# smdogroup/eigd

Measured on AMD Instinct MI355X. Metric: adjoint_mode_derivatives_per_sec, higher is better.
Workload: dtype f64

## Files before the change

eigd_amd/csrc/factor.hip:

```cpp
#include <algorithm>
#include <cstdlib>
#include <cstring>
#include <mutex>

#include "common.h"
#include "symbolic.h"

struct eigd_symbolic {
  eigd::Symbolic s;
  std::mutex upper_lock;
};

static bool ensure_upper_map(eigd_symbolic* h) {
  std::lock_guard<std::mutex> g(h->upper_lock);
  return eigd::build_upper_map(h->s);
}

namespace eigd {

constexpr int TW = 64;
constexpr int TLD = TW + 1;
constexpr int kFragWavesFwd = 2, kFragWaves = 3, kFragWavesBwd32 = 2, kThinWavesLeaf = 3, kThinWavesKids = 1;
constexpr int KBMAX = 32;

struct FrontArrays {
  const int* c0;
  const int* ns;
  const int* bs;
  const int* parent;
  const int64_t* foff;
  const int64_t* voff;
  const int64_t* ioff;
  const int64_t* bptr;
  const int* rel;
  const int64_t* toff;
  int nslot;
  int64_t vrows;
  const int* v_src;
  const int* cmask;
  const int* bout;
  double* sgn;
  const double* zero;
  const int* neg1;
  int W;
  int tri;
  double pivtol;
};

constexpr int kPlaneCols = 4 + 8 + 16 + 32;
constexpr int kMaxS = 4;

__device__ __forceinline__ int find_slot(const int* __restrict__ pref, int na, int idx) {
  int lo = 0, hi = na;
  while (hi - lo > 1) {
    const int mid = (lo + hi) >> 1;
    if (pref[mid] <= idx)
      lo = mid;
    else
      hi = mid;
  }
  return lo;
}

__global__ void scatter_a_kernel(int64_t nlower, const int64_t* __restrict__ src, const int64_t* __restrict__ dst,
                                 const double* __restrict__ data, double* __restrict__ F) {
  for (int64_t e = static_cast<int64_t>(blockIdx.x) * blockDim.x + threadIdx.x; e < nlower;
       e += static_cast<int64_t>(gridDim.x) * blockDim.x)
    F[dst[e]] = data[src[e]];
}

__global__ __launch_bounds__(kThreads) void absmax_kernel(int64_t n, const double* __restrict__ x, double* __restrict__ partial) {
  __shared__ double red[kThreads];
  double m = 0.0;
  for (int64_t i = static_cast<int64_t>(blockIdx.x) * kThreads + threadIdx.x; i < n; i += static_cast<int64_t>(gridDim.x) * kThreads)
    m = fmax(m, fabs(x[i]));
  red[threadIdx.x] = m;
  __syncthreads();
  for (int s = kThreads / 2; s > 0; s >>= 1) {
    if (threadIdx.x < s) red[threadIdx.x] = fmax(red[threadIdx.x], red[threadIdx.x + s]);
    __syncthreads();
  }
  if (threadIdx.x == 0) partial[blockIdx.x] = red[0];
}

__global__ __launch_bounds__(kThreads) void extend_add_kernel(FrontArrays fa, const int* __restrict__ children,
                                                             double* __restrict__ F) {
  const int c = children[blockIdx.x];
  const int p = fa.parent[c];
  const int ns = fa.ns[c], bs = fa.bs[c];
  const int64_t dc = ns + bs, dp = fa.ns[p] + fa.bs[p];
  const int* __restrict__ rel = fa.rel + fa.bptr[c];
  const double* __restrict__ Fc = F + fa.foff[c] + static_cast<int64_t>(ns) * dc + ns;
  double* Fp = F + fa.foff[p];
  const int total = bs * bs;
  for (int idx = blockIdx.y * kThreads + threadIdx.x; idx < total; idx += gridDim.y * kThreads) {
    const int j = idx / bs, i = idx - j * bs;
    if (i >= j) Fp[static_cast<int64_t>(rel[j]) * dp + rel[i]] += Fc[static_cast<int64_t>(j) * dc + i];
  }
}

__global__ __launch_bounds__(kThreads) void potrf_inv_kernel(FrontArrays fa, const int* __restrict__ fronts, int step,
                                                            double* __restrict__ F, double* __restrict__ Inv,
                                                            int* __restrict__ flag) {
  __shared__ double S[TW * TLD];
  __shared__ double Iv[TW * TLD];
// ... 569 lines not shown
    }
    __syncthreads();
    double out[4][4];
#pragma unroll
    for (int p = 0; p < 4; ++p)
#pragma unroll
      for (int q = 0; q < 4; ++q) out[p][q] = 0.0;
    for (int kk = 0; kk < wi; ++kk) {
      double a[4], b[4];
#pragma unroll
      for (int q = 0; q < 4; ++q) a[q] = As[kk * TLD + r0 + q];
#pragma unroll
      for (int q = 0; q < 4; ++q) b[q] = Bs[kk * TLD + c0 + q];
#pragma unroll
      for (int p = 0; p < 4; ++p)
#pragma unroll
        for (int q = 0; q < 4; ++q) out[p][q] += a[p] * b[q];
    }
#pragma unroll
    for (int q = 0; q < 4; ++q)
#pragma unroll
      for (int p = 0; p < 4; ++p)
        if (r0 + p < wi && c0 + q < wj) Tf[static_cast<int64_t>(j0 + c0 + q) * ns + i0 + r0 + p] = -out[p][q];
    __threadfence();
    __syncthreads();
  }
}

__global__ __launch_bounds__(kThreads) void m21_kernel(FrontArrays fa, const int* __restrict__ m_pref, int nfronts,
                                                      double* F, const double* __restrict__ Tb) {
  __shared__ double As[TW * TLD];
  __shared__ double Bs[TW * TLD];
  const int f = find_slot(m_pref, nfronts, blockIdx.x);
  const int bt = blockIdx.x - m_pref[f];
  const int ns = fa.ns[f];
  const int64_t d = ns + fa.bs[f];
  const int rb0 = ns + bt * TW;
  const int rows = min(TW, static_cast<int>(d) - rb0);
  const int nct = (ns + TW - 1) / TW;
  double* Ff = F + fa.foff[f];
  const double* Tf = Tb + fa.toff[f];
  const int tid = threadIdx.x;
  const int r0 = (tid % 16) * 4, c0 = (tid / 16) * 4;
  for (int jt = 0; jt < nct; ++jt) {
    const int j0 = jt * TW, wj = min(TW, ns - j0);
    double acc[4][4];
#pragma unroll
    for (int a = 0; a < 4; ++a)
#pragma unroll
      for (int b = 0; b < 4; ++b) acc[a][b] = 0.0;
    for (int kt = jt; kt < nct; ++kt) {
      const int k0 = kt * TW, wk = min(TW, ns - k0);
      for (int idx = tid; idx < TW * TW; idx += kThreads) {
        const int kk = idx / TW, r = idx - kk * TW;
        As[kk * TLD + r] = (kk < wk && r < rows) ? Ff[static_cast<int64_t>(k0 + kk) * d + rb0 + r] : 0.0;
      }
      for (int idx = tid; idx < TW * TW; idx += kThreads) {
        const int c = idx / TW, kk = idx - c * TW;
        Bs[kk * TLD + c] = (kk < wk && c < wj) ? Tf[static_cast<int64_t>(j0 + c) * ns + k0 + kk] : 0.0;
      }
      __syncthreads();
      for (int kk = 0; kk < wk; ++kk) {
        double a[4], b[4];
#pragma unroll
        for (int q = 0; q < 4; ++q) a[q] = As[kk * TLD + r0 + q];
#pragma unroll
        for (int q = 0; q < 4; ++q) b[q] = Bs[kk * TLD + c0 + q];
#pragma unroll
        for (int p = 0; p < 4; ++p)
#pragma unroll
          for (int q = 0; q < 4; ++q) acc[p][q] += a[p] * b[q];
      }
      __syncthreads();
    }
#pragma unroll
    for (int q = 0; q < 4; ++q)
#pragma unroll
      for (int p = 0; p < 4; ++p)
        if (r0 + p < rows && c0 + q < wj) Ff[static_cast<int64_t>(j0 + c0 + q) * d + rb0 + r0 + p] = acc[p][q];
  }
}


template <int KPT>
struct Tile {
  static constexpr bool kMfma = (KPT >= 4);
  static constexpr int KB = 4 * KPT;
  static constexpr int NT = kMfma ? KB / 16 : 1;
  static constexpr int BLD = (KB == 32) ? 48 : KB;
  static constexpr int NOUT = kMfma ? 4 * NT : KPT;

  __device__ static __forceinline__ void coords(int t, int& row, int& col) {
    if (kMfma) {
      const int lane = threadIdx.x & 63, wave = threadIdx.x >> 6;
      row = 16 * wave + (lane >> 4) + 4 * (t & 3);
      col = 16 * (t >> 2) + (lane & 15);
    } else {
      row = threadIdx.x >> 2;
      col = (threadIdx.x & 3) * KPT + t;
    }
  }

  __device__ static __forceinline__ void mac(const double* __restrict__ As, const double* __restrict__ Bs, int kdim,
                                             double (&acc)[NOUT]) {
    if constexpr (kMfma) {
      const int lane = threadIdx.x & 63, wave = threadIdx.x >> 6;
      const int li = lane & 15, lk = lane >> 4;
      const int o = 16 * wave + li;
      double4_t c[NT];
#pragma unroll
      for (int n = 0; n < NT; ++n) c[n] = double4_t{acc[4 * n], acc[4 * n + 1], acc[4 * n + 2], acc[4 * n + 3]};
      const int kd = (kdim + 7) & ~7;
      for (int k0 = 0; k0 < kd; k0 += 8) {
#pragma unroll
        for (int kk = 0; kk < 8; kk += 4) {
          const int k = k0 + kk + lk;
          const double a = As[k * TLD + o];
#pragma unroll
          for (int n = 0; n < NT; ++n)
            c[n] = __builtin_amdgcn_mfma_f64_16x16x4f64(a, Bs[k * BLD + 16 * n + li], c[n], 0, 0, 0);
        }
      }
#pragma unroll
      for (int n = 0; n < NT; ++n)
#pragma unroll
        for (int r = 0; r < 4; ++r) acc[4 * n + r] = c[n][r];
    } else {
      const int o = threadIdx.x >> 2, cg = threadIdx.x & 3;
      const int kd = (kdim + 7) & ~7;
      for (int k0 = 0; k0 < kd; k0 += 8) {
#pragma unroll
        for (int kk = 0; kk < 8; ++kk) {
          const int k = k0 + kk;
          const double a = As[k * TLD + o];
          const double* b = Bs + k * BLD + cg * KPT;
#pragma unroll
          for (int q = 0; q < KPT; ++q) acc[q] += a * b[q];
        }
      }
    }
  }
};

struct WgRec {
  int f, tile, s0, s1;
  int slab, cnt, G, flags;
  int ns, bs, c0, slot;
  int64_t voff, foff, toff, bptr;
  int64_t pvoff;
  int64_t scratch;
  int64_t ftoff;
  int64_t ldt;
  int64_t moff;
};

struct FragFront {
  int f, nst, nbt, nko;
  int nkb, pad;
  int64_t fm, bm;
};

__device__ __host__ inline int64_t frag_fwd_steps(int nst, int nko, int rt) {
  const int64_t ks = 16 * (nst - 1) + nko;
  return (rt <= nst - 1) ? 8LL * rt * (rt + 1) : 8LL * (nst - 1) * nst + ks * (rt - (nst - 1));
}
__device__ __host__ inline int64_t frag_bwd_chain(int nst, int nbt, int nko, int nkb, int ct) {
// ... 1 lines not shown
}
__device__ __host__ inline int64_t frag_bwd_steps(int nst, int nbt, int nko, int nkb, int ct) {
  int64_t sum = 0;
  for (int c = 0; c < ct; ++c) sum += frag_bwd_chain(nst, nbt, nko, nkb, c);
  return sum;
}
__device__ __host__ inline int64_t frag_bwd_in_chain(int nown, int nko, int t) {
  return (t < nown) ? 16LL * t : 16LL * (nown - 1) + nko + 16LL * (t - nown);
}

struct LevelArgs {
  const WgRec* wg;
  double* P;
  int* tickets;
  int kb;
  int kd;
  int nwg;
  int per_xcd;
  double* V1;
};

__device__ __forceinline__ int xcd_record(const LevelArgs& la) {
  if (la.per_xcd == 0) return blockIdx.x;
  return (blockIdx.x & 7) * la.per_xcd + (blockIdx.x >> 3);
}

constexpr int TILE_IT = TW * TW / kThreads;

__global__ void overflow_sum_kernel(int nrows, const int* __restrict__ ov_dst, const int* __restrict__ ov_ptr,
                                    const int* __restrict__ ov_src, int kb, int ld, double* __restrict__ extra,
                                    const double* __restrict__ scratch) {
  const int idx = blockIdx.x * blockDim.x + threadIdx.x;
  if (idx >= nrows * kb) return;
  const int x = idx / kb, c = idx - x * kb;
  double sum = 0.0;
  for (int e = ov_ptr[x]; e < ov_ptr[x + 1]; ++e) sum += scratch[static_cast<int64_t>(ov_src[e]) * ld + c];
  extra[static_cast<int64_t>(ov_dst[x]) * ld + c] = sum;
}

template <int KPT>
__device__ __forceinline__ bool fold_groups(const WgRec& w, const LevelArgs& la, double (&acc)[Tile<KPT>::NOUT],
                                            int* sflag) {
  using T = Tile<KPT>;
  typedef unsigned long long u64;
  double* Pp = la.P + static_cast<int64_t>(w.slab) * (TW * KBMAX);
  u64* mine = reinterpret_cast<u64*>(Pp + static_cast<int64_t>(w.flags >> 8) * (TW * KBMAX));
#pragma unroll
  for (int t = 0; t < T::NOUT; ++t)
    __hip_atomic_store(mine + t * kThreads + threadIdx.x, static_cast<u64>(__double_as_longlong(acc[t])),
                       __ATOMIC_RELAXED, __HIP_MEMORY_SCOPE_AGENT);
  asm volatile("s_waitcnt vmcnt(0)" ::: "memory");
  __syncthreads();
  if (threadIdx.x == 0)
    *sflag = (__hip_atomic_fetch_add(la.tickets + w.cnt, 1, __ATOMIC_RELAXED, __HIP_MEMORY_SCOPE_AGENT) == w.G - 1) ? 1 : 0;
  __syncthreads();
  if (*sflag == 0) return false;
  if (threadIdx.x == 0) {
    __hip_atomic_store(la.tickets + w.cnt, 0, __ATOMIC_RELAXED, __HIP_MEMORY_SCOPE_AGENT);
    __builtin_amdgcn_fence(__ATOMIC_ACQUIRE, "agent");
    asm volatile("s_waitcnt vmcnt(0)" ::: "memory");
  }
  __syncthreads();
#pragma unroll
  for (int t = 0; t < T::NOUT; ++t) acc[t] = 0.0;
  for (int gg = 0; gg < w.G; gg += 2) {
    const double* p0 = Pp + static_cast<int64_t>(gg) * (TW * KBMAX) + threadIdx.x;
    const bool two = gg + 1 < w.G;
    double a[T::NOUT], b[T::NOUT];
#pragma unroll
    for (int t = 0; t < T::NOUT; ++t) {
      a[t] = p0[t * kThreads];
      b[t] = two ? p0[TW * KBMAX + t * kThreads] : 0.0;
    }
#pragma unroll
    for (int t = 0; t < T::NOUT; ++t) {
      acc[t] += a[t];
      if (two) acc[t] += b[t];
    }
  }
  return true;
}

template <int KPT, bool SINGLE, int NSL, bool FRAG = false, bool PRE = false>
__global__ __launch_bounds__(kThreads) __attribute__((amdgpu_waves_per_eu(((SINGLE && KPT >= 4) || (FRAG && KPT >= 4)) ? ((FRAG && KPT >= 8) ? kFragWavesFwd : 3) : 1)))
void fwd_level_kernel(FrontArrays fa, LevelArgs la, const double* __restrict__ F,
                                                            const double* __restrict__ Tb, const double* X, int ldx,
                                                            double alpha, double* V, double* __restrict__ Y) {
  using T = Tile<KPT>;
  constexpr int IT = KPT;
  extern __shared__ double lds_tiles[];
  double* const As = lds_tiles;
  const int kdl = SINGLE ? la.kd : TW;
  double* const Bs = lds_tiles + (((SINGLE && KPT == 4) || FRAG) ? 0 : (kdl + 1) * TLD);
  const int rec = SINGLE ? static_cast<int>(blockIdx.x) : xcd_record(la);
  if (!SINGLE && rec >= la.nwg) return;
  const WgRec w = la.wg[rec];
  const int kb = la.kb;
  const int ns = w.ns;
  const int d = ns + w.bs;
  const int nst = (ns + TW - 1) / TW;
  const bool kids = (w.flags & 2) != 0;
  const int64_t vbase = w.voff;
  const double* Tf = Tb + w.toff;
  const double* Ff = F + w.foff;
  const int ar = threadIdx.x & (TW - 1), ajb = threadIdx.x >> 6;

  int xi[IT];
  double bv[IT], av[TILE_IT];
  const int nslot = kids ? fa.nslot : 0;
  const int64_t vslot = fa.vrows * T::KB;
  double* Vout = V + static_cast<int64_t>(w.slot) * vslot;

  static_assert(!PRE || FRAG, "pre-assembled right-hand sides: the fragment path only");
  auto fetch_idx = [&](int ct) {
    if constexpr (PRE) return;
    const int wd = min(TW, ns - ct * TW);
#pragma unroll
    for (int e = 0; e < IT; ++e) {
      const int r = (threadIdx.x + e * kThreads) / T::KB;
      const int64_t vrow = vbase + ct * TW + r;
      const bool ok = r < wd;
      xi[e] = *(ok ? fa.v_src + vrow : fa.neg1);
    }
  };
  auto fetch_b = [&](int ct) {
    if constexpr (PRE) {
      const int wd = min(TW, ns - ct * TW);
      const double* V1 = la.V1 + (vbase + ct * TW) * T::KB;
#pragma unroll
      for (int e = 0; e < IT; ++e) {
        const int idx = threadIdx.x + e * kThreads;
        bv[e] = *(((idx & (T::KB - 1)) < kb && idx / T::KB < wd) ? V1 + idx : fa.zero);
      }
      return;
    }
#pragma unroll
    for (int e = 0; e < IT; ++e) {
      const int idx = threadIdx.x + e * kThreads;
      const int c = idx & (T::KB - 1);
      const bool ok = c < kb && xi[e] >= 0;
      const double xv = alpha * *(ok ? X + static_cast<int64_t>(xi[e]) * ldx + c : fa.zero);
      const double* cp = V + (vbase + ct * TW + idx / T::KB) * T::KB + c;
      double v = 0.0;
#pragma unroll
      for (int s = 0; s < NSL; ++s) v += *((ok && s < nslot) ? cp + s * vslot : fa.zero);
      bv[e] = xv + v;
    }
  };
  auto fetch_a = [&](int rt, int ct, double (&av)[TILE_IT]) {
    const bool own = rt < nst;
    const int row0 = own ? rt * TW : ns + (rt - nst) * TW;
    const int rows = min(TW, (own ? ns : d) - row0);
    const int64_t ld = own ? w.ldt : d;
    const int wd = min(TW, ns - ct * TW);
    const double* Ap = (own ? Tf : Ff) + static_cast<int64_t>(ct) * TW * ld + row0 + ar;
#pragma unroll
    for (int it = 0; it < TILE_IT; ++it) {
      const int j = ajb + it * (kThreads / TW);
      av[it] = *((j < wd && ar < rows) ? Ap + static_cast<int64_t>(j) * ld : fa.zero);
    }
  };
  auto commit_a = [&](const double (&av)[TILE_IT]) {
#pragma unroll
    for (int it = 0; it < TILE_IT; ++it)
      As[min(ajb + it * (kThreads / TW), kdl) * TLD + ar] = av[it];
  };
  auto commit_b = [&]() {
// ... 74 lines not shown
      const double* Ab = (own ? Tf : Ff) + row0;
      const ptrdiff_t zoff = fa.zero - Ab;
#pragma unroll
      for (int kk = 0; kk < 16; ++kk) {
        const int k = 4 * kk + lk;
        a[kk] = (k < ns && orow < rows) ? Ab[static_cast<unsigned>(k * ld + orow)] : Ab[zoff];
      }
    };
    auto stepd = [&](int rt, double (&cur)[16], int nxt) {
      if (KPT < 8 && rt >= nst) fetch_carry(rt, cg, di);
      double4_t c[T::NT];
#pragma unroll
      for (int n = 0; n < T::NT; ++n) c[n] = double4_t{0.0, 0.0, 0.0, 0.0};
#pragma unroll
      for (int kk = 0; kk < 16; ++kk) {
        const int k = 4 * kk + lk;
#pragma unroll
        for (int n = 0; n < T::NT; ++n)
          c[n] = __builtin_amdgcn_mfma_f64_16x16x4f64(cur[kk], Bs[k * T::BLD + 16 * n + li], c[n], 0, 0, 0);
      }
      if (nxt < w.s1) fetch_frag(nxt, cur);
#pragma unroll
      for (int n = 0; n < T::NT; ++n)
#pragma unroll
        for (int r = 0; r < 4; ++r) acc[4 * n + r] = c[n][r];
      if (KPT >= 8 && rt >= nst) fetch_carry(rt, cg, di);
      store_tile(rt, acc, cg, di);
    };
    double a0[16];
    fetch_idx(0);
    fetch_frag(w.s0, a0);
    constexpr int HB = (IT > 4) ? IT / 2 : IT;
#pragma unroll
    for (int h = 0; h < IT; h += HB) {
      double vh[HB];
#pragma unroll
      for (int e = h; e < h + HB; ++e) {
        const int idx = threadIdx.x + e * kThreads;
        const int c = idx & (T::KB - 1);
        const bool ok = c < kb && xi[e] >= 0;
        const double xv = alpha * *(ok ? X + static_cast<int64_t>(xi[e]) * ldx + c : fa.zero);
        const double* cp = V + (vbase + idx / T::KB) * T::KB + c;
        double v = 0.0;
#pragma unroll
        for (int s = 0; s < NSL; ++s) v += *((ok && s < nslot) ? cp + s * vslot : fa.zero);
        vh[e - h] = xv + v;
      }
#pragma unroll
      for (int e = h; e < h + HB; ++e) {
        const int idx = threadIdx.x + e * kThreads;
        Bs[min(idx / T::KB, kdl) * T::BLD + (idx & (T::KB - 1))] = vh[e - h];
      }
      asm volatile("" ::: "memory");
    }
    __syncthreads();
    for (int rt = w.s0; rt < w.s1; ++rt) stepd(rt, a0, rt + 1);
  } else if constexpr (SINGLE) {
    auto step = [&](int rt, double (&cur)[TILE_IT], int nxt) {
      commit_a(cur);
      __syncthreads();
      if (nxt < w.s1) fetch_a(nxt, 0, cur);
      if (rt >= nst) fetch_carry(rt, cg, di);
#pragma unroll
      for (int t = 0; t < T::NOUT; ++t) acc[t] = 0.0;
      T::mac(As, Bs, ns, acc);
      store_tile(rt, acc, cg, di);
      __syncthreads();
    };
    fetch_idx(0);
    fetch_b(0);
    fetch_a(w.s0, 0, av);
    commit_b();
    for (int rt = w.s0; rt < w.s1; ++rt) step(rt, av, rt + 1);
  } else if constexpr (FRAG) {
    static_assert(!FRAG || T::kMfma, "fragments feed MFMAs");
    const int wave = threadIdx.x >> 6, lane = threadIdx.x & 63;
    const int li = lane & 15, lk = lane >> 4;
    const int rt = w.tile;
    const bool own = rt < nst;
    const int row0 = own ? rt * TW : ns + (rt - nst) * TW;
    const int rows = min(TW, (own ? ns : d) - row0);
    const bool wok = 16 * wave < rows;
    const double* Am = F + w.moff + wave * 64 + lane;
    auto fetch_frag = [&](int ct, double (&a)[16]) {
      const int nk = (min(TW, ns - ct * TW) + 3) >> 2;
      const double* Ac = Am + static_cast<int64_t>(ct) * (TW * TW);
#pragma unroll
      for (int kk = 0; kk < 16; ++kk) a[kk] = (wok && kk < nk) ? Ac[kk * 256] : 0.0;
    };
    double4_t c[T::NT];
#pragma unroll
    for (int n = 0; n < T::NT; ++n) c[n] = double4_t{0.0, 0.0, 0.0, 0.0};
    auto stepf = [&](int ct, double (&cur)[16], double (&nxt)[16]) {
      commit_b();
      __syncthreads();
      if (ct + 1 < w.s1) {
        fetch_b(ct + 1);
        fetch_frag(ct + 1, nxt);
        if (ct + 2 < w.s1) fetch_idx(ct + 2);
      }
      const int nk = (min(TW, ns - ct * TW) + 3) >> 2;
#pragma unroll
      for (int kk = 0; kk < 16; ++kk) {
        if (kk < nk) {
          const int k = 4 * kk + lk;
#pragma unroll
          for (int n = 0; n < T::NT; ++n)
            c[n] = __builtin_amdgcn_mfma_f64_16x16x4f64(cur[kk], Bs[k * T::BLD + 16 * n + li], c[n], 0, 0, 0);
        }
      }
      __syncthreads();
    };
    double a0[16], a1[16];
    fetch_frag(w.s0, a0);
    fetch_idx(w.s0);
    fetch_b(w.s0);
    if (w.s0 + 1 < w.s1) fetch_idx(w.s0 + 1);
    for (int ct = w.s0; ct < w.s1; ct += 2) {
      stepf(ct, a0, a1);
      if (ct + 1 < w.s1) stepf(ct + 1, a1, a0);
    }
#pragma unroll
    for (int n = 0; n < T::NT; ++n)
#pragma unroll
      for (int r = 0; r < 4; ++r) acc[4 * n + r] = c[n][r];
    if (rt >= nst) fetch_carry(rt, cg, di);
    if (w.G > 1 && !fold_groups<KPT>(w, la, acc, reinterpret_cast<int*>(Bs))) return;
    store_tile(rt, acc, cg, di);
  } else {
  const int rt = w.tile;
  fetch_idx(w.s0);
  fetch_b(w.s0);
  fetch_a(rt, w.s0, av);
  if (w.s0 + 1 < w.s1) fetch_idx(w.s0 + 1);
  for (int ct = w.s0; ct < w.s1; ++ct) {
    commit_a(av);
    commit_b();
    __syncthreads();
    if (ct + 1 < w.s1) {
      fetch_b(ct + 1);
      fetch_a(rt, ct + 1, av);
      if (ct + 2 < w.s1) fetch_idx(ct + 2);
    }
    T::mac(As, Bs, min(TW, ns - ct * TW), acc);
    __syncthreads();
  }
  if (rt >= nst) fetch_carry(rt, cg, di);
  if (w.G > 1 && !fold_groups<KPT>(w, la, acc, reinterpret_cast<int*>(As))) return;
  store_tile(rt, acc, cg, di);
  }
}

template <int KPT, int NSL>
__global__ __launch_bounds__(kThreads) void v1_assemble_kernel(FrontArrays fa, const WgRec* __restrict__ recs, const double* X,
                                                              int ldx, double alpha, const double* V, double* V1p, int kb) {
  using T = Tile<KPT>;
  constexpr int IT = KPT;
  const WgRec w = recs[blockIdx.x];
  const int ct = w.tile;
  const int wd = min(TW, w.ns - ct * TW);
  const int64_t vrow0 = w.voff + ct * TW;
  const int nslot = ((w.flags & 2) != 0) ? fa.nslot : 0;
  const int64_t vslot = fa.vrows * T::KB;
  int xi[IT];
#pragma unroll
  for (int e = 0; e < IT; ++e) {
    const int r = (threadIdx.x + e * kThreads) / T::KB;
    xi[e] = *((r < wd) ? fa.v_src + vrow0 + r : fa.neg1);
  }
  double bv[IT];
#pragma unroll
  for (int e = 0; e < IT; ++e) {
    const int idx = threadIdx.x + e * kThreads;
    const int c = idx & (T::KB - 1);
    const bool ok = c < kb && xi[e] >= 0;
    const double xv = alpha * *(ok ? X + static_cast<int64_t>(xi[e]) * ldx + c : fa.zero);
    const double* cp = V + vrow0 * T::KB + idx;
    double v = 0.0;
#pragma unroll
    for (int s = 0; s < NSL; ++s) v += *((ok && s < nslot) ? cp + s * vslot : fa.zero);
    bv[e] = xv + v;
  }
  double* V1 = V1p + vrow0 * T::KB;
#pragma unroll
  for (int e = 0; e < IT; ++e) {
    const int idx = threadIdx.x + e * kThreads;
    if ((idx & (T::KB - 1)) < kb && xi[e] >= 0) V1[idx] = bv[e];
  }
}

constexpr int kLidxMax = 7168;
template <int KPT, bool SINGLE, bool FRAG = false, bool LIDX = false>
__global__ __launch_bounds__(kThreads) __attribute__((amdgpu_waves_per_eu(FRAG ? (KPT >= 8 ? (LIDX ? 3 : kFragWavesBwd32) : kFragWaves) : 1)))
void bwd_level_kernel(FrontArrays fa, LevelArgs la, const double* __restrict__ F,
                                                            const double* __restrict__ Tb, const double* __restrict__ Ft,
                                                            const double* __restrict__ Y, double* Out, int ldo) {
  using T = Tile<KPT>;
  constexpr int IT = KPT;
  extern __shared__ double lds_tiles[];
  double* const As = lds_tiles;
  const int kdl = SINGLE ? la.kd : TW;
  double* const Bs = lds_tiles + (FRAG ? 0 : (kdl + 1) * TLD);
  const int rec = SINGLE ? static_cast<int>(blockIdx.x) : xcd_record(la);
  if (!SINGLE && rec >= la.nwg) return;
  const WgRec w = la.wg[rec];
  const int ct = w.tile;
  const int kb = la.kb;
  const int ns = w.ns, bs = w.bs;
  const int d = ns + bs;
  const int nst = (ns + TW - 1) / TW;
  const int c0t = ct * TW;
  const int wc = min(TW, ns - c0t);
  const int nown = nst - ct;
  const int64_t vbase = w.voff;
  const double* Tp = Tb + w.toff + static_cast<int64_t>(c0t) * w.ldt;
  const double* Mp = F + w.foff + static_cast<int64_t>(c0t) * d;
  const int* __restrict__ bout = fa.bout + w.bptr;
  const int ar = threadIdx.x & (TW - 1), ajb = threadIdx.x >> 6;

  int ri[IT];
  double bv[IT], av[TILE_IT];
  int pend_rows = 0;

  auto fetch_idx = [&](int t) {
    if (t < nown) return;
    const int b0 = (t - nown) * TW;
    const int rows = min(TW, bs - b0);
#pragma unroll
    for (int e = 0; e < IT; ++e) {
      const int r = (threadIdx.x + e * kThreads) / T::KB;
      ri[e] = *((r < rows) ? bout + b0 + r : fa.neg1);
    }
  };
  auto fetch_val = [&](int t) {
    const bool border = t >= nown;
    const int rbase = border ? ns + (t - nown) * TW : (ct + t) * TW;
    const int rows = min(TW, (border ? d : ns) - rbase);
    if (!border) {
      const double* Yp = Y + (vbase + rbase) * kb;
#pragma unroll
      for (int e = 0; e < IT; ++e) {
        const int idx = threadIdx.x + e * kThreads;
        const int r = idx / T::KB, c = idx & (T::KB - 1);
        bv[e] = *((r < rows && c < kb) ? Yp + static_cast<int64_t>(r) * kb + c : fa.zero);
      }
    } else {
#pragma unroll
      for (int e = 0; e < IT; ++e) {
        const int c = (threadIdx.x + e * kThreads) & (T::KB - 1);
        bv[e] = -*((ri[e] >= 0 && c < kb) ? Out + static_cast<int64_t>(ri[e]) * ldo + c : fa.zero);
      }
    }
    const double* Ap = (border ? Mp : Tp) + rbase + ar;
    const int64_t ld = border ? d : w.ldt;
#pragma unroll
    for (int it = 0; it < TILE_IT; ++it) {
      const int j = ajb + it * (kThreads / TW);
      av[it] = *((j < wc && ar < rows) ? Ap + static_cast<int64_t>(j) * ld : fa.zero);
    }
    pend_rows = rows;
  };
  auto commit = [&]() {
#pragma unroll
    for (int it = 0; it < TILE_IT; ++it)
      As[min(ar, kdl) * TLD + ajb + it * (kThreads / TW)] = av[it];
#pragma unroll
    for (int e = 0; e < IT; ++e) {
      const int idx = threadIdx.x + e * kThreads;
      Bs[min(idx / T::KB, kdl) * T::BLD + (idx & (T::KB - 1))] = bv[e];
    }
  };

  double acc[T::NOUT];
  int oi[T::NOUT];
#pragma unroll
  for (int t = 0; t < T::NOUT; ++t) acc[t] = 0.0;
  if constexpr (FRAG) {
    static_assert(!FRAG || (!SINGLE && T::kMfma), "fragments: several column tiles, MFMA widths");
    const int wave = threadIdx.x >> 6, lane = threadIdx.x & 63;
    const int li = lane & 15, lk = lane >> 4;
    const bool wok = 16 * wave < wc;
    const int nko = (ns - TW * (nst - 1) + 3) >> 2;
    const double* Am = Ft + w.moff + wave * 64 + lane;
    int frag_rows = 0;
    static_assert(!LIDX || FRAG, "index list in LDS: the fragment path only");
    int* const Is = reinterpret_cast<int*>(Bs + (TW + 1) * T::BLD);
    auto fetch_vec = [&](int t) {
      const bool border = t >= nown;
      const int rbase = border ? ns + (t - nown) * TW : (ct + t) * TW;
      const int rows = min(TW, (border ? d : ns) - rbase);
      if (!border) {
        const double* Yp = Y + (vbase + rbase) * kb;
#pragma unroll
        for (int e = 0; e < IT; ++e) {
          const int idx = threadIdx.x + e * kThreads;
          const int r = idx / T::KB, c = idx & (T::KB - 1);
          bv[e] = *((r < rows && c < kb) ? Yp + static_cast<int64_t>(r) * kb + c : fa.zero);
        }
      } else if constexpr (LIDX) {
        const int b0 = (t - nown) * TW;
        int rr[IT];
#pragma unroll
        for (int e = 0; e < IT; ++e) {
          const int r = (threadIdx.x + e * kThreads) / T::KB;
          rr[e] = (r < rows) ? Is[b0 + r] : -1;
        }
#pragma unroll
        for (int e = 0; e < IT; ++e) {
          const int c = (threadIdx.x + e * kThreads) & (T::KB - 1);
          bv[e] = -*((rr[e] >= 0 && c < kb) ? Out + static_cast<int64_t>(rr[e]) * ldo + c : fa.zero);
        }
      } else {
#pragma unroll
        for (int e = 0; e < IT; ++e) {
          const int c = (threadIdx.x + e * kThreads) & (T::KB - 1);
          bv[e] = -*((ri[e] >= 0 && c < kb) ? Out + static_cast<int64_t>(ri[e]) * ldo + c : fa.zero);
        }
      }
    };
    auto fetch_frag = [&](int t, double (&a)[16]) {
      const bool border = t >= nown;
      const int rbase = border ? ns + (t - nown) * TW : (ct + t) * TW;
      const int rows = min(TW, (border ? d : ns) - rbase);
      const int nk = (rows + 3) >> 2;
      const double* Ac = Am + 256 * frag_bwd_in_chain(nown, nko, t);
#pragma unroll
      for (int kk = 0; kk < 16; ++kk) a[kk] = (wok && kk < nk) ? Ac[kk * 256] : 0.0;
      frag_rows = rows;
    };
    auto commit_vec = [&]() {
#pragma unroll
      for (int e = 0; e < IT; ++e) {
        const int idx = threadIdx.x + e * kThreads;
        Bs[(idx / T::KB) * T::BLD + (idx & (T::KB - 1))] = bv[e];
      }
    };
    double4_t c[T::NT];
#pragma unroll
    for (int n = 0; n < T::NT; ++n) c[n] = double4_t{0.0, 0.0, 0.0, 0.0};
    auto stepb = [&](int t, double (&cur)[16], double (&nxt)[16]) {
      const int nk = (frag_rows + 3) >> 2;
      commit_vec();
      __syncthreads();
      if (t + 1 < w.s1) {
        fetch_vec(t + 1);
        fetch_frag(t + 1, nxt);
        if (!LIDX && t + 2 < w.s1) fetch_idx(t + 2);
      }
#pragma unroll
      for (int kk = 0; kk < 16; ++kk) {
        if (kk < nk) {
          const int k = 4 * kk + lk;
#pragma unroll
          for (int n = 0; n < T::NT; ++n)
            c[n] = __builtin_amdgcn_mfma_f64_16x16x4f64(cur[kk], Bs[k * T::BLD + 16 * n + li], c[n], 0, 0, 0);
        }
      }
      __syncthreads();
    };
    double a0[16], a1[16];
    fetch_frag(w.s0, a0);
    if constexpr (LIDX) {
      constexpr int NI = 8;
      int ib[NI];
      const bool any = w.s1 > nown;
#pragma unroll
      for (int q = 0; q < NI; ++q) ib[q] = *((any && threadIdx.x + q * kThreads < bs) ? bout + threadIdx.x + q * kThreads : fa.neg1);
      if (w.s0 < nown) fetch_vec(w.s0);
#pragma unroll
      for (int q = 0; q < NI; ++q)
        if (any && threadIdx.x + q * kThreads < bs) Is[threadIdx.x + q * kThreads] = ib[q];
      if (any)
        for (int i = NI * kThreads + threadIdx.x; i < bs; i += kThreads) Is[i] = bout[i];
      if (w.s0 >= nown) {
        __syncthreads();
        fetch_vec(w.s0);
      }
    } else {
      fetch_idx(w.s0);
      fetch_vec(w.s0);
      if (w.s0 + 1 < w.s1) fetch_idx(w.s0 + 1);
    }
    for (int t = w.s0; t < w.s1; t += 2) {
      stepb(t, a0, a1);
      if (t + 1 < w.s1) stepb(t + 1, a1, a0);
    }
#pragma unroll
    for (int n = 0; n < T::NT; ++n)
#pragma unroll
      for (int r = 0; r < 4; ++r) acc[4 * n + r] = c[n][r];
  } else {
  fetch_idx(w.s0);
  fetch_val(w.s0);
  if (w.s0 + 1 < w.s1) fetch_idx(w.s0 + 1);
  for (int t = w.s0; t < w.s1; ++t) {
    const int kdim = pend_rows;
    commit();
    __syncthreads();
    if (t + 1 < w.s1) {
      fetch_val(t + 1);
      if (t + 2 < w.s1) fetch_idx(t + 2);
    }
    T::mac(As, Bs, kdim, acc);
    __syncthreads();
  }
  }
#pragma unroll
  for (int t = 0; t < T::NOUT; ++t) {
    int o, c;
    T::coords(t, o, c);
    oi[t] = *((o < wc && c < kb) ? fa.v_src + vbase + c0t + o : fa.neg1);
  }
  if (w.G > 1 && !fold_groups<KPT>(w, la, acc, reinterpret_cast<int*>(lds_tiles))) return;
  __builtin_amdgcn_s_waitcnt(0x0F70);
#pragma unroll
  for (int t = 0; t < T::NOUT; ++t) {
    int o, c;
    T::coords(t, o, c);
    if (oi[t] >= 0) Out[static_cast<int64_t>(oi[t]) * ldo + c] = acc[t];
  }
}

__device__ __forceinline__ double readlane_f64(double v, int l) {
  const int lo = __builtin_amdgcn_readlane(__double2loint(v), l);
  const int hi = __builtin_amdgcn_readlane(__double2hiint(v), l);
  return __hiloint2double(hi, lo);
}

template <int KB, int NSL, int WPF>
__global__ __launch_bounds__(64 * WPF) void fwd_wave_kernel(FrontArrays fa, const WgRec* __restrict__ recs,
                                                       const double* __restrict__ F, const double* __restrict__ Tb,
                                                       const double* X, int ldx, double alpha, double* V,
                                                       double* __restrict__ Y, int kb) {
  const WgRec w = recs[blockIdx.x];
  const int lane = threadIdx.x & 63, wave = threadIdx.x >> 6;
  const int ns = w.ns, d = ns + w.bs;
  const bool kids = (w.flags & 2) != 0;
  const int nslot = kids ? fa.nslot : 0;
  const int64_t vslot = fa.vrows * KB, vbase = w.voff;
  double b[KB];
  {
// ... 1085 lines not shown
      upload_buffer("f_bptr", f->d_bptr, s.f_bptr),
      upload_buffer("lvl_fronts", f->d_lvl_fronts, s.lvl_fronts),
      upload_buffer("pref_chunks", f->d_pref_chunks, s.pref_chunks),
      upload_buffer("pref_tiles", f->d_pref_tiles, s.pref_tiles),
      upload_buffer("fwd_wg", f->d_fwd_wg, p.fwd_wg),
      upload_buffer("bwd_wg", f->d_bwd_wg, p.bwd_wg),
      upload_buffer("wave_wg", f->d_wave_wg, p.wave_wg),
      upload_buffer("pre_wg", f->d_pre_wg, p.pre_wg),
      upload_buffer("ftoff", f->d_ftoff, p.ftoff),
      upload_buffer("tr_pref", f->d_tr_pref, p.tr_pref),
      upload_buffer("mt_pref", f->d_mt_pref, p.mt_pref)};
  if (!p.ffr.empty()) t.push_back(upload_buffer("ffr", f->d_ff, p.ffr));
  t.insert(t.end(), {upload_buffer("bout", f->d_bout, p.bout),
                     upload_buffer("tri_pref", f->d_tri_pref, p.tri_pref),
                     upload_buffer("m_pref", f->d_m_pref, p.m_pref),
                     upload_buffer("toff", f->d_toff, p.toff),
                     upload_buffer("ov_dst", f->d_ov_dst, p.ov_dst),
                     upload_buffer("ov_ptr", f->d_ov_ptr, p.ov_ptr),
                     upload_buffer("ov_src", f->d_ov_src, p.ov_src),
                     upload_buffer("cs_child", f->d_cs_child, s.cs_child),
                     upload_buffer("a_src", f->L.src, s.a_src),
                     upload_buffer("a_dst", f->L.dst, s.a_dst),
                     upload_buffer("v_src", f->d_v_src, s.v_src)});
  if (f->lu) t.insert(t.end(), {upload_buffer("u_src", f->U.src, s.u_src), upload_buffer("u_dst", f->U.dst, s.u_dst)});
  t.insert(t.end(), {upload_buffer("cmask", f->d_cmask, p.cmask),
                     device_buffer("data", f->d_data, f->data_len),
                     device_buffer("F", f->L.F, s.front_doubles),
                     device_buffer("Inv", f->L.Inv, s.inv_doubles, true),
                     device_buffer("T", f->L.T, p.t_doubles, true),
                     DeviceBuffer{"aux", reinterpret_cast<void**>(&f->d_aux), sizeof(double), 2, false, aux},
                     device_buffer("red", f->d_red, 512),
                     device_buffer("Ft", f->L.Ft, p.ft_doubles),
                     device_buffer("Fb", f->d_Fb, p.ft_doubles),
                     device_buffer("Fm", f->d_Fm, p.fm_doubles),
                     device_buffer("Bm", f->L.Bm, p.bm_doubles)});
  const std::vector<DeviceBuffer> ws = workspace_buffers(f->ws, *f);
  t.insert(t.end(), ws.begin(), ws.end());
  t.push_back(device_buffer("sgn", f->d_sgn, s.n));
  if (f->lu)
    t.insert(t.end(), {device_buffer("FU", f->U.F, s.front_doubles),
                       device_buffer("InvU", f->U.Inv, s.inv_doubles, true),
                       device_buffer("TU", f->U.T, p.t_doubles, true),
                       device_buffer("FtU", f->U.Ft, p.ft_doubles),
                       device_buffer("BmU", f->U.Bm, p.bm_doubles)});
  t.push_back(device_buffer("flag", f->d_flag, 4));
  return t;
}

constexpr int kWaveMaxKpt = 2;

#define EIGD_UNPAREN(...) __VA_ARGS__
#define EIGD_SWEEP_LAUNCH(KERNEL, TARGS, ...)                                                               \
  do {                                                                                                      \
    if (rec) rec->launches.push_back({SweepVariant<KERNEL##_family, EIGD_UNPAREN TARGS>::id, l, kb});      \
    hipLaunchKernelGGL((KERNEL<EIGD_UNPAREN TARGS>), __VA_ARGS__);                                         \
  } while (0)

template <int KPT>
int sweep(eigd_factor* f, const SweepCopies& cp, hipStream_t st, const SweepWorkspace& ws, const double* dIn, int ldin,
          double* dX, int ldx, int kb, double alpha, SweepRecord* rec) {
  double *wV = ws.V, *wY = ws.Y, *wP = ws.P;
  int* wT = ws.tickets;
  const Symbolic& s = *f->sym;
  const FrontArrays fa = f->fa();
  constexpr int KB = 4 * KPT;
  const int ncarry = f->nplanes - (f->has_v1 ? 1 : 0);
  double* const wV1 = f->has_v1 ? wV + static_cast<int64_t>(ncarry) * f->v_rows * kPlaneCols + f->v_rows * (KB - 4) : nullptr;
  wV += static_cast<int64_t>(ncarry) * f->v_rows * (KB - 4);
  auto level_args = [&](const WgRec* wg, int kd = TW, int nwg = 0, bool multi = false) {
    LevelArgs la;
    la.wg = wg;
    la.P = wP;
    la.tickets = wT;
    la.kb = kb;
    la.kd = kd;
    la.nwg = nwg;
    la.per_xcd = multi ? (nwg + 7) / 8 : 0;
    la.V1 = wV1;
    return la;
  };
  auto multi_grid = [&](int nwg) { return dim3(8 * ((nwg + 7) / 8)); };
  auto lds_bytes = [](int kd) { return static_cast<unsigned>(sizeof(double) * (kd + 1) * (TLD + Tile<KPT>::BLD)); };
  const unsigned lds_frag = static_cast<unsigned>(sizeof(double) * (TW + 1) * Tile<KPT>::BLD);
  const double* sF = cp.fF;
  const double* sT = cp.fT;
  const bool thin_buf = f->v_rows * static_cast<int64_t>(KB) * 8 <= kBufMax && static_cast<int64_t>(s.n) * ldin * 8 <= kBufMax;
  for (int l = 0; l < s.nlevels; ++l) {
    const int nov = f->ov_lvl_ptr[l + 1] - f->ov_lvl_ptr[l];
    if (nov > 0) {
      const int first = f->ov_lvl_ptr[l];
      const int64_t plane = f->v_rows * KB;
      if (rec) rec->launches.push_back({SweepVariant<overflow_sum_kernel_family>::id, l, kb});
      hipLaunchKernelGGL(overflow_sum_kernel, dim3((nov * kb + 255) / 256), dim3(256), 0, st, nov, f->d_ov_dst + first,
                         f->d_ov_ptr + first, f->d_ov_src, kb, KB, wV + (f->nslot - 1) * plane, wV + f->nslot * plane);
      EIGD_LAUNCH_CHECK();
    }
    const int nwg = f->h_fwd_ptr[l + 1] - f->h_fwd_ptr[l], nsingle = f->h_fwd_nsingle[l];
    const bool two = f->h_lvl_two[l] != 0;
    const bool leaf = f->h_lvl_leaf[l] != 0;
    const int nwave = f->h_wave_ptr[l + 1] - f->h_wave_ptr[l];
    bool narrow = false;
    if (KPT <= kWaveMaxKpt) {
      if (nwave > 0) {
        const WgRec* recs = f->d_wave_wg + f->h_wave_ptr[l];
        if (leaf)
          EIGD_SWEEP_LAUNCH(fwd_wave_kernel, (KB, 0, 2), dim3(nwave), dim3(128), 0, st, fa, recs, sF, sT, dIn, ldin, alpha, wV,
                             wY, kb);
        else if (two)
          EIGD_SWEEP_LAUNCH(fwd_wave_kernel, (KB, 2, 2), dim3(nwave), dim3(128), 0, st, fa, recs, sF, sT, dIn, ldin, alpha, wV,
                             wY, kb);
        else
          EIGD_SWEEP_LAUNCH(fwd_wave_kernel, (KB, kMaxS + 1, 2), dim3(nwave), dim3(128), 0, st, fa, recs, sF, sT, dIn, ldin,
                             alpha, wV, wY, kb);
        EIGD_LAUNCH_CHECK();
        narrow = true;
      }
    }
    if constexpr (KPT >= 4) {
      const int nks = f->h_thin_fwd[l];
      if (!narrow && nwave > 0 && nks > 0 && thin_buf) {
        const WgRec* recs = f->d_wave_wg + f->h_wave_ptr[l];
#define EIGD_THIN_FWD(NKS, NSLV, WPFV)                                                                                   \
  do {                                                                                                                   \
    if (fa.tri)                                                                                                          \
      EIGD_SWEEP_LAUNCH(fwd_thin_kernel, (KB, NKS, NSLV, WPFV, true), dim3(nwave), dim3(64 * WPFV), 0, st, fa, recs, dIn, ldin, \
                         alpha, wV, wY, kb, cp.Fb);                                                                    \
    else                                                                                                                 \
      EIGD_SWEEP_LAUNCH(fwd_thin_kernel, (KB, NKS, NSLV, WPFV, false), dim3(nwave), dim3(64 * WPFV), 0, st, fa, recs, dIn, ldin, \
                         alpha, wV, wY, kb, cp.Fb);                                                                    \
  } while (0)
        if (!leaf && two && nks >= 12) {
          const int wpf = (nwave >= 2048) ? 1 : (nwave >= 1024) ? 2 : 4;
          if (nks == 12 && wpf == 1)
            EIGD_THIN_FWD(12, 2, 1);
          else if (nks == 12 && wpf == 2)
            EIGD_THIN_FWD(12, 2, 2);
          else if (nks == 12)
            EIGD_THIN_FWD(12, 2, 4);
          else if (wpf == 1)
            EIGD_THIN_FWD(16, 2, 1);
          else if (wpf == 2)
            EIGD_THIN_FWD(16, 2, 2);
          else
            EIGD_THIN_FWD(16, 2, 4);
        } else if (leaf && nks == 4)
          EIGD_THIN_FWD(4, 0, 1);
        else if (leaf && nks == 8)
          EIGD_THIN_FWD(8, 0, 1);
        else if (leaf && nks == 12)
          EIGD_THIN_FWD(12, 0, 1);
        else if (leaf && nks == 14)
          EIGD_THIN_FWD(14, 0, 1);
        else if (leaf)
          EIGD_THIN_FWD(16, 0, 1);
        else if (nks == 4 && two)
          EIGD_THIN_FWD(4, 2, 1);
        else if (nks == 4)
          EIGD_THIN_FWD(4, kMaxS + 1, 1);
        else if (nks == 8 && two)
          EIGD_THIN_FWD(8, 2, 1);
        else if (nks == 8)
          EIGD_THIN_FWD(8, kMaxS + 1, 1);
        else if (two)
          EIGD_THIN_FWD(16, 2, 1);
        else
          EIGD_THIN_FWD(16, kMaxS + 1, 1);
#undef EIGD_THIN_FWD
        EIGD_LAUNCH_CHECK();
        narrow = true;
      }
    }
    if (!narrow && nsingle > 0) {
      const int kd = (KPT == 4) ? TW : f->h_fwd_kd[l];
      const LevelArgs la = level_args(f->d_fwd_wg + f->h_fwd_ptr[l], kd);
      auto lds_bytes = [](int kd) {
        return static_cast<unsigned>(sizeof(double) * (kd + 1) * ((KPT == 4 ? 0 : TLD) + Tile<KPT>::BLD));
      };
      if (leaf)
        EIGD_SWEEP_LAUNCH(fwd_level_kernel, (KPT, true, 0, false, false), dim3(nsingle), dim3(kThreads), lds_bytes(kd), st, fa, la,
                           sF, sT, dIn, ldin, alpha, wV, wY);
      else if (two)
        EIGD_SWEEP_LAUNCH(fwd_level_kernel, (KPT, true, 2, false, false), dim3(nsingle), dim3(kThreads), lds_bytes(kd), st, fa, la,
                           sF, sT, dIn, ldin, alpha, wV, wY);
      else
        EIGD_SWEEP_LAUNCH(fwd_level_kernel, (KPT, true, kMaxS + 1, false, false), dim3(nsingle), dim3(kThreads), lds_bytes(kd), st,
                           fa, la, sF, sT, dIn, ldin, alpha, wV, wY);
      EIGD_LAUNCH_CHECK();
    }
    if (nwg > nsingle) {
      const LevelArgs la = level_args(f->d_fwd_wg + f->h_fwd_ptr[l] + nsingle, TW, nwg - nsingle, true);
      if constexpr (Tile<KPT>::kMfma) {
        const int npre = f->h_pre_ptr[l + 1] - f->h_pre_ptr[l];
        if (npre > 0) {
          const WgRec* pre = f->d_pre_wg + f->h_pre_ptr[l];
          if (two) {
            EIGD_SWEEP_LAUNCH(v1_assemble_kernel, (KPT, 2), dim3(npre), dim3(kThreads), 0, st, fa, pre, dIn, ldin, alpha, wV,
                               wV1, kb);
            EIGD_SWEEP_LAUNCH(fwd_level_kernel, (KPT, false, 2, true, true), multi_grid(nwg - nsingle), dim3(kThreads),
                               lds_frag, st, fa, la, cp.Fm, sT, dIn, ldin, alpha, wV, wY);
          } else {
            EIGD_SWEEP_LAUNCH(v1_assemble_kernel, (KPT, kMaxS + 1), dim3(npre), dim3(kThreads), 0, st, fa, pre, dIn, ldin,
                               alpha, wV, wV1, kb);
            EIGD_SWEEP_LAUNCH(fwd_level_kernel, (KPT, false, kMaxS + 1, true, true), multi_grid(nwg - nsingle),
                               dim3(kThreads), lds_frag, st, fa, la, cp.Fm, sT, dIn, ldin, alpha, wV, wY);
          }
        } else if (two)
          EIGD_SWEEP_LAUNCH(fwd_level_kernel, (KPT, false, 2, true, false), multi_grid(nwg - nsingle), dim3(kThreads),
                             lds_frag, st, fa, la, cp.Fm, sT, dIn, ldin, alpha, wV, wY);
        else
          EIGD_SWEEP_LAUNCH(fwd_level_kernel, (KPT, false, kMaxS + 1, true, false), multi_grid(nwg - nsingle),
                             dim3(kThreads), lds_frag, st, fa, la, cp.Fm, sT, dIn, ldin, alpha, wV, wY);
      } else {
        if (two)
          EIGD_SWEEP_LAUNCH(fwd_level_kernel, (KPT, false, 2, false, false), multi_grid(nwg - nsingle), dim3(kThreads),
                             lds_bytes(TW), st, fa, la, sF, sT, dIn, ldin, alpha, wV, wY);
        else
          EIGD_SWEEP_LAUNCH(fwd_level_kernel, (KPT, false, kMaxS + 1, false, false), multi_grid(nwg - nsingle), dim3(kThreads),
                             lds_bytes(TW), st, fa, la, sF, sT, dIn, ldin, alpha, wV, wY);
      }
      EIGD_LAUNCH_CHECK();
    }
  }
  for (int l = s.nlevels - 1; l >= 0; --l) {
    const int nwg = f->h_bwd_ptr[l + 1] - f->h_bwd_ptr[l];
    if (nwg == 0) continue;
    const int nwave = f->h_wave_ptr[l + 1] - f->h_wave_ptr[l];
    const int nsb = f->h_bwd_nsingle[l];
    const bool narrow = KPT <= kWaveMaxKpt && nwave > 0;
    bool thin = false;
    if constexpr (KPT >= 4) thin = !narrow && nwave > 0 && f->h_thin_bwd[l] > 0;
    if (nwg > nsb) {
      const LevelArgs la = level_args(f->d_bwd_wg + f->h_bwd_ptr[l] + nsb, TW, nwg - nsb, true);
      if constexpr (Tile<KPT>::kMfma) {
        if (KPT >= 8 && f->h_bwd_mxbs[l] <= kLidxMax)
          EIGD_SWEEP_LAUNCH(bwd_level_kernel, (KPT, false, true, (KPT >= 8)), multi_grid(nwg - nsb), dim3(kThreads),
                             lds_frag + 4u * static_cast<unsigned>((f->h_bwd_mxbs[l] + 3) & ~3), st, fa, la, cp.bF, cp.bT, cp.Bm,
                             wY, dX, ldx);
        else
          EIGD_SWEEP_LAUNCH(bwd_level_kernel, (KPT, false, true, false), multi_grid(nwg - nsb), dim3(kThreads), lds_frag, st, fa,
                             la, cp.bF, cp.bT, cp.Bm, wY, dX, ldx);
      }
      else
        EIGD_SWEEP_LAUNCH(bwd_level_kernel, (KPT, false, false, false), multi_grid(nwg - nsb), dim3(kThreads), lds_bytes(TW), st, fa, la, cp.bF,
                           cp.bT, cp.Ft, wY, dX, ldx);
      EIGD_LAUNCH_CHECK();
    }
    if (narrow) {
      EIGD_SWEEP_LAUNCH(bwd_wave_kernel, (KB), dim3(nwave), dim3(64), 0, st, fa, f->d_wave_wg + f->h_wave_ptr[l], cp.Ft,
                         wY, dX, ldx, kb);
      EIGD_LAUNCH_CHECK();
    } else if (thin) {
      if constexpr (KPT >= 4) {
        const WgRec* recs = f->d_wave_wg + f->h_wave_ptr[l];
        const int nks = f->h_thin_bwd[l];
#define EIGD_THIN_BWD(NOB, CHV)                                                                                   \
  do {                                                                                                            \
    if (fa.tri)                                                                                                   \
      EIGD_SWEEP_LAUNCH(bwd_thin_kernel, (KB, NOB, CHV, true), dim3(nwave), dim3(64), 0, st, fa, recs, cp.Ft, wY, \
                         dX, ldx, kb);                                                                            \
    else                                                                                                          \
      EIGD_SWEEP_LAUNCH(bwd_thin_kernel, (KB, NOB, CHV, false), dim3(nwave), dim3(64), 0, st, fa, recs, cp.Ft, \
                         wY, dX, ldx, kb);                                                                        \
  } while (0)
        if (nks == 4)
          EIGD_THIN_BWD(1, 8);
        else if (nks == 8)
          EIGD_THIN_BWD(2, 8);
        else
          EIGD_THIN_BWD(4, 4);
#undef EIGD_THIN_BWD
        EIGD_LAUNCH_CHECK();
      }
    } else if (nsb > 0) {
      EIGD_SWEEP_LAUNCH(bwd_level_kernel, (KPT, true, false, false), dim3(nsb), dim3(kThreads), lds_bytes(f->h_bwd_kd[l]), st, fa,
                         level_args(f->d_bwd_wg + f->h_bwd_ptr[l], f->h_bwd_kd[l]), cp.bF, cp.bT, cp.Ft, wY, dX, ldx);
      EIGD_LAUNCH_CHECK();
    }
  }
  return EIGD_OK;
}
#undef EIGD_SWEEP_LAUNCH
#undef EIGD_UNPAREN

}

extern "C" {

int eigd_symbolic_create(int n, const int32_t* hindptr, const int32_t* hindices, int leaf_size, int panel_width,
                         eigd_symbolic** out) {
  return eigd_symbolic_create_geom(n, hindptr, hindices, leaf_size, panel_width, 0, nullptr, out);
}

int eigd_symbolic_create_geom(int n, const int32_t* hindptr, const int32_t* hindices, int leaf_size, int panel_width,
                              int dim, const double* hcoords, eigd_symbolic** out) {
  EIGD_REQUIRE(hindptr && hindices && out, "null argument");
  EIGD_REQUIRE(hcoords == nullptr || (dim >= 1 && dim <= 3), "coordinates need 1 <= dim <= 3");
  *out = nullptr;
  eigd_symbolic* h = new eigd_symbolic();
  if (!analyze(n, hindptr, hindices, leaf_size, panel_width, h->s, dim, hcoords)) {
    set_error("symbolic analysis failed: %s", h->s.error.c_str());
    delete h;
    return EIGD_E_INVALID;
  }
  *out = h;
  return EIGD_OK;
}

int eigd_symbolic_free(eigd_symbolic* s) {
  delete s;
  return EIGD_OK;
}

int eigd_symbolic_sizes(eigd_symbolic* h, int64_t* out, int nout) {
  EIGD_REQUIRE(h && out && nout >= 1, "null argument");
  const Symbolic& s = h->s;
  const int64_t v[12] = {s.n,
                         s.nfronts,
                         s.nlevels,
                         s.nnzL,
                         s.front_doubles,
                         s.sumd,
                         s.maxd,
// ... 239 lines not shown
```

Measured before the change: 683.6.

## Stage part of the MFMA A fragments through LDS via direct global-to-LDS loads

In the fragment paths of the forward and backward level kernels, the first NKL k-steps of each A fragment are now loaded with global_load_lds straight into a per-wave LDS region and read back right before the MFMAs, instead of being held in registers across the prefetch. This cuts VGPR pressure, so the waves-per-EU hint for those variants rises from 2 to 3, and the LDS allocation per launch grows to hold the staged steps. In exchange it adds an explicit vmcnt(0) wait before each step and replaces the closing __syncthreads with a hand-written lgkmcnt wait plus barrier, which could expose load latency or cause ordering problems.

```diff
diff --git a/eigd_amd/csrc/factor.hip b/eigd_amd/csrc/factor.hip
--- a/eigd_amd/csrc/factor.hip
+++ b/eigd_amd/csrc/factor.hip
@@ -20,7 +20,19 @@
 
 constexpr int TW = 64;
 constexpr int TLD = TW + 1;
-constexpr int kFragWavesFwd = 2, kFragWaves = 3, kFragWavesBwd32 = 2, kThinWavesLeaf = 3, kThinWavesKids = 1;
+constexpr int kThinWavesLeaf = 3, kThinWavesKids = 1;
+#ifndef EIGD_FRAG_REGS
+#define EIGD_FRAG_REGS 0
+#endif
+#if EIGD_FRAG_REGS
+template <int KPT, bool PRE> constexpr int kFwdLdsSteps = 0;
+template <int KPT, bool LIDX> constexpr int kBwdLdsSteps = 0;
+#else
+template <int KPT, bool PRE> constexpr int kFwdLdsSteps = (KPT >= 8) ? (PRE ? 12 : 0) : (PRE ? 8 : 12);
+template <int KPT, bool LIDX> constexpr int kBwdLdsSteps = (KPT >= 8 && !LIDX) ? 12 : 0;
+#endif
+constexpr int kFragWavesFwd = 2, kFragWaves = 3, kFragWavesBwd32 = 2;
+constexpr int kFragStepBytes = 2048;
 constexpr int KBMAX = 32;
 
 struct FrontArrays {
@@ -756,6 +768,22 @@
 }
 
 
+__device__ __forceinline__ void load_to_lds16(const double* src, double* dst) {
+  __builtin_amdgcn_global_load_lds((const __attribute__((address_space(1))) void*)src,
+                                   (__attribute__((address_space(3))) void*)dst, 16, 0, 0);
+}
+template <int NKL>
+__device__ __forceinline__ void frag_to_lds(const double* tile, int nk, double* Ls) {
+  const int lane = threadIdx.x & 63;
+  const int hi = lane >> 5;
+  const unsigned lo = 2u * (lane & 31);
+#pragma unroll
+  for (int j = 0; j < NKL / 2; ++j) {
+    const int kk = 2 * j + hi;
+    load_to_lds16(tile + ((kk < nk ? kk : 0) * 256u + lo), Ls + j * 128);
+  }
+}
+
 template <int KPT>
 struct Tile {
   static constexpr bool kMfma = (KPT >= 4);
@@ -923,7 +951,7 @@
 }
 
 template <int KPT, bool SINGLE, int NSL, bool FRAG = false, bool PRE = false>
-__global__ __launch_bounds__(kThreads) __attribute__((amdgpu_waves_per_eu(((SINGLE && KPT >= 4) || (FRAG && KPT >= 4)) ? ((FRAG && KPT >= 8) ? kFragWavesFwd : 3) : 1)))
+__global__ __launch_bounds__(kThreads) __attribute__((amdgpu_waves_per_eu(((SINGLE && KPT >= 4) || (FRAG && KPT >= 4)) ? ((FRAG && KPT >= 8) ? (kFwdLdsSteps<KPT, PRE> > 0 ? 3 : kFragWavesFwd) : 3) : 1)))
 void fwd_level_kernel(FrontArrays fa, LevelArgs la, const double* __restrict__ F,
                                                             const double* __restrict__ Tb, const double* X, int ldx,
                                                             double alpha, double* V, double* __restrict__ Y) {
@@ -1164,16 +1192,29 @@
     const int rows = min(TW, (own ? ns : d) - row0);
     const bool wok = 16 * wave < rows;
     const double* Am = F + w.moff + wave * 64 + lane;
+    constexpr int NKL = kFwdLdsSteps<KPT, PRE>;
+    const int uwave = __builtin_amdgcn_readfirstlane(wave);
+    double* const Ls = Bs + (TW + 1) * T::BLD + uwave * (NKL * 64);
+    const double* const Au = F + w.moff + uwave * 64;
     auto fetch_frag = [&](int ct, double (&a)[16]) {
       const int nk = (min(TW, ns - ct * TW) + 3) >> 2;
       const double* Ac = Am + static_cast<int64_t>(ct) * (TW * TW);
-#pragma unroll
-      for (int kk = 0; kk < 16; ++kk) a[kk] = (wok && kk < nk) ? Ac[kk * 256] : 0.0;
+      if constexpr (NKL > 0) frag_to_lds<NKL>(Au + (Ac - Am), nk, Ls);
+#pragma unroll
+      for (int kk = NKL; kk < 16; ++kk) a[kk] = (wok && kk < nk) ? Ac[kk * 256] : 0.0;
+    };
+    auto take_frag = [&](double (&a)[16]) {
+      if constexpr (NKL > 0) {
+        asm volatile("s_waitcnt vmcnt(0)" ::: "memory");
+#pragma unroll
+        for (int kk = 0; kk < NKL; ++kk) a[kk] = Ls[kk * 64 + lane];
+      }
     };
     double4_t c[T::NT];
 #pragma unroll
     for (int n = 0; n < T::NT; ++n) c[n] = double4_t{0.0, 0.0, 0.0, 0.0};
     auto stepf = [&](int ct, double (&cur)[16], double (&nxt)[16]) {
+      take_frag(cur);
       commit_b();
       __syncthreads();
       if (ct + 1 < w.s1) {
@@ -1191,7 +1232,8 @@
             c[n] = __builtin_amdgcn_mfma_f64_16x16x4f64(cur[kk], Bs[k * T::BLD + 16 * n + li], c[n], 0, 0, 0);
         }
       }
-      __syncthreads();
+      if constexpr (NKL > 0) asm volatile("s_waitcnt lgkmcnt(0)\n\ts_barrier" ::: "memory");
+      else __syncthreads();
     };
     double a0[16], a1[16];
     fetch_frag(w.s0, a0);
@@ -1273,7 +1315,7 @@
 
 constexpr int kLidxMax = 7168;
 template <int KPT, bool SINGLE, bool FRAG = false, bool LIDX = false>
-__global__ __launch_bounds__(kThreads) __attribute__((amdgpu_waves_per_eu(FRAG ? (KPT >= 8 ? (LIDX ? 3 : kFragWavesBwd32) : kFragWaves) : 1)))
+__global__ __launch_bounds__(kThreads) __attribute__((amdgpu_waves_per_eu(FRAG ? (KPT >= 8 ? ((LIDX || kBwdLdsSteps<KPT, LIDX> > 0) ? 3 : kFragWavesBwd32) : kFragWaves) : 1)))
 void bwd_level_kernel(FrontArrays fa, LevelArgs la, const double* __restrict__ F,
                                                             const double* __restrict__ Tb, const double* __restrict__ Ft,
                                                             const double* __restrict__ Y, double* Out, int ldo) {
@@ -1367,6 +1409,11 @@
     int frag_rows = 0;
     static_assert(!LIDX || FRAG, "index list in LDS: the fragment path only");
     int* const Is = reinterpret_cast<int*>(Bs + (TW + 1) * T::BLD);
+    constexpr int NKL = kBwdLdsSteps<KPT, LIDX>;
+    static_assert(!LIDX || NKL == 0, "the index list and the fragments would share the space behind the vector block");
+    const int uwave = __builtin_amdgcn_readfirstlane(wave);
+    double* const Ls = Bs + (TW + 1) * T::BLD + uwave * (NKL * 64);
+    const double* const Au = Ft + w.moff + uwave * 64;
     auto fetch_vec = [&](int t) {
       const bool border = t >= nown;
       const int rbase = border ? ns + (t - nown) * TW : (ct + t) * TW;
@@ -1406,9 +1453,17 @@
       const int rows = min(TW, (border ? d : ns) - rbase);
       const int nk = (rows + 3) >> 2;
       const double* Ac = Am + 256 * frag_bwd_in_chain(nown, nko, t);
-#pragma unroll
-      for (int kk = 0; kk < 16; ++kk) a[kk] = (wok && kk < nk) ? Ac[kk * 256] : 0.0;
+      if constexpr (NKL > 0) frag_to_lds<NKL>(Au + (Ac - Am), nk, Ls);
+#pragma unroll
+      for (int kk = NKL; kk < 16; ++kk) a[kk] = (wok && kk < nk) ? Ac[kk * 256] : 0.0;
       frag_rows = rows;
+    };
+    auto take_frag = [&](double (&a)[16]) {
+      if constexpr (NKL > 0) {
+        asm volatile("s_waitcnt vmcnt(0)" ::: "memory");
+#pragma unroll
+        for (int kk = 0; kk < NKL; ++kk) a[kk] = Ls[kk * 64 + lane];
+      }
     };
     auto commit_vec = [&]() {
 #pragma unroll
@@ -1422,6 +1477,7 @@
     for (int n = 0; n < T::NT; ++n) c[n] = double4_t{0.0, 0.0, 0.0, 0.0};
     auto stepb = [&](int t, double (&cur)[16], double (&nxt)[16]) {
       const int nk = (frag_rows + 3) >> 2;
+      take_frag(cur);
       commit_vec();
       __syncthreads();
       if (t + 1 < w.s1) {
@@ -1438,7 +1494,8 @@
             c[n] = __builtin_amdgcn_mfma_f64_16x16x4f64(cur[kk], Bs[k * T::BLD + 16 * n + li], c[n], 0, 0, 0);
         }
       }
-      __syncthreads();
+      if constexpr (NKL > 0) asm volatile("s_waitcnt lgkmcnt(0)\n\ts_barrier" ::: "memory");
+      else __syncthreads();
     };
     double a0[16], a1[16];
     fetch_frag(w.s0, a0);
@@ -2690,6 +2747,8 @@
   auto multi_grid = [&](int nwg) { return dim3(8 * ((nwg + 7) / 8)); };
   auto lds_bytes = [](int kd) { return static_cast<unsigned>(sizeof(double) * (kd + 1) * (TLD + Tile<KPT>::BLD)); };
   const unsigned lds_frag = static_cast<unsigned>(sizeof(double) * (TW + 1) * Tile<KPT>::BLD);
+  const unsigned lds_fwd = lds_frag + kFragStepBytes * kFwdLdsSteps<KPT, false>, lds_fwd_pre = lds_frag + kFragStepBytes * kFwdLdsSteps<KPT, true>;
+  const unsigned lds_bwd = lds_frag + kFragStepBytes * kBwdLdsSteps<KPT, false>;
   const double* sF = cp.fF;
   const double* sT = cp.fT;
   const bool thin_buf = f->v_rows * static_cast<int64_t>(KB) * 8 <= kBufMax && static_cast<int64_t>(s.n) * ldin * 8 <= kBufMax;
@@ -2805,19 +2864,19 @@
             EIGD_SWEEP_LAUNCH(v1_assemble_kernel, (KPT, 2), dim3(npre), dim3(kThreads), 0, st, fa, pre, dIn, ldin, alpha, wV,
                                wV1, kb);
             EIGD_SWEEP_LAUNCH(fwd_level_kernel, (KPT, false, 2, true, true), multi_grid(nwg - nsingle), dim3(kThreads),
-                               lds_frag, st, fa, la, cp.Fm, sT, dIn, ldin, alpha, wV, wY);
+                               lds_fwd_pre, st, fa, la, cp.Fm, sT, dIn, ldin, alpha, wV, wY);
           } else {
             EIGD_SWEEP_LAUNCH(v1_assemble_kernel, (KPT, kMaxS + 1), dim3(npre), dim3(kThreads), 0, st, fa, pre, dIn, ldin,
                                alpha, wV, wV1, kb);
             EIGD_SWEEP_LAUNCH(fwd_level_kernel, (KPT, false, kMaxS + 1, true, true), multi_grid(nwg - nsingle),
-                               dim3(kThreads), lds_frag, st, fa, la, cp.Fm, sT, dIn, ldin, alpha, wV, wY);
+                               dim3(kThreads), lds_fwd_pre, st, fa, la, cp.Fm, sT, dIn, ldin, alpha, wV, wY);
           }
         } else if (two)
           EIGD_SWEEP_LAUNCH(fwd_level_kernel, (KPT, false, 2, true, false), multi_grid(nwg - nsingle), dim3(kThreads),
-                             lds_frag, st, fa, la, cp.Fm, sT, dIn, ldin, alpha, wV, wY);
+                             lds_fwd, st, fa, la, cp.Fm, sT, dIn, ldin, alpha, wV, wY);
         else
           EIGD_SWEEP_LAUNCH(fwd_level_kernel, (KPT, false, kMaxS + 1, true, false), multi_grid(nwg - nsingle),
-                             dim3(kThreads), lds_frag, st, fa, la, cp.Fm, sT, dIn, ldin, alpha, wV, wY);
+                             dim3(kThreads), lds_fwd, st, fa, la, cp.Fm, sT, dIn, ldin, alpha, wV, wY);
       } else {
         if (two)
           EIGD_SWEEP_LAUNCH(fwd_level_kernel, (KPT, false, 2, false, false), multi_grid(nwg - nsingle), dim3(kThreads),
@@ -2845,7 +2904,7 @@
                              lds_frag + 4u * static_cast<unsigned>((f->h_bwd_mxbs[l] + 3) & ~3), st, fa, la, cp.bF, cp.bT, cp.Bm,
                              wY, dX, ldx);
         else
-          EIGD_SWEEP_LAUNCH(bwd_level_kernel, (KPT, false, true, false), multi_grid(nwg - nsb), dim3(kThreads), lds_frag, st, fa,
+          EIGD_SWEEP_LAUNCH(bwd_level_kernel, (KPT, false, true, false), multi_grid(nwg - nsb), dim3(kThreads), lds_bwd, st, fa,
                              la, cp.bF, cp.bT, cp.Bm, wY, dX, ldx);
       }
       else
```

Result: no change. 682.9, median of 3 (-0.1%).
